# bluescarni/heyoka

Hardware: AMD Instinct MI355X
Metric: ODE systems x steps/sec (fp64) (higher is better)
Workload: dtype f64

## Files before the change

### heyoka_amd/csrc/hip_emit_cluster2.cpp

```cpp
#include <algorithm>
#include <cstdio>
#include <functional>

#include "hip_emit_cluster2_gen.hpp"
#include "logging.hpp"

namespace heyoka_amd::cluster2_detail
{

cluster2_gen::cluster2_gen(const taylor_program &p_, const emit_options &opts_, std::string &why_not_, bool allow_one_lane_,
                           std::uint32_t min_lanes_)
    : c2_emit(p_, opts_.order), p(p_), opts(opts_), why_not(why_not_), allow_one_lane(allow_one_lane_), min_lanes(min_lanes_),
      n_eq(p_.n_eq), order(opts_.order)
{
    std::string s = opts.dev.v5_opts;
    std::replace(s.begin(), s.end(), '+', ',');
    for (std::size_t b = 0, en = 0; b <= s.size(); b = en + 1u) {
        en = std::min(s.find(',', b), s.size());
        v5_flags.insert(s.substr(b, en - b));
    }
}

cluster2_attempt cluster2_gen::run()
{
// ... 93 lines not shown
            for (std::uint32_t i = 0; i < 3u; ++i) {
                pl.slot_of[pl.clusters[c][static_cast<std::uint32_t>(pp.rx[i])]] = static_cast<int>(ns++);
            }
        }
        number_glue_slots(ns);
    }
    L = pl.L, spw = pl.spw;
    bs = pairk ? 512u : 256u;
    wpb = bs / 64u;
    n_ext = static_cast<std::uint32_t>(pl.ext_u[0].size());
    n_out = static_cast<std::uint32_t>(pl.out_pos.size());
    n_cst = static_cast<std::uint32_t>(pl.cst_pos.size());

    variant = one_lane ? cluster2_variant::one_lane : (pair_split ? cluster2_variant::lane_pair : cluster2_variant::pipelined);
    frx = false;
    if (one_lane && !m4 && pp.rx[0] >= 0 && pl.groups.size() == 1u && !v5_flag("nofrx")) {
        auto &nodes = pl.groups[0].nodes;
        std::map<std::uint32_t, bool> is_rx_out;
        for (std::uint32_t c = 0; c < nc; ++c) {
            for (std::uint32_t i = 0; i < 3u; ++i) {
                is_rx_out[pl.clusters[c][pp.pr[i]]] = false;
                is_rx_out[pl.clusters[c][static_cast<std::uint32_t>(pp.rx[i])]] = true;
            }
        }
        const auto &n0 = p.nodes[nodes[0] - n_eq];
        frx = n0.kind == func_kind::sum && n0.args.size() >= 2u;
        std::vector<char> plain(nodes.size(), 1);
        for (std::size_t j = 0; j < nodes.size() && frx; ++j) {
            const auto &nd = p.nodes[nodes[j] - n_eq];
            frx = nd.kind == func_kind::sum && nd.args.size() == n0.args.size();
            for (const auto &o : nd.args) {
                const auto it = is_var(o) ? is_rx_out.find(o.idx) : is_rx_out.end();
                frx = frx && it != is_rx_out.end();
                if (frx && it->second) {
                    plain[j] = 0;
                }
            }
        }
        if (frx) {
            std::vector<std::uint32_t> first, last;
            for (std::size_t j = 0; j < nodes.size(); ++j) {
                (plain[j] != 0 ? last : first).push_back(nodes[j]);
            }
            frx = first.size() <= pl.L && !last.empty();
            if (frx) {
                first.insert(first.end(), last.begin(), last.end());
                nodes = std::move(first);
            }
        }
    }
}

void cluster2_gen::anchors_and_reaction_fusion()
{
    std::vector<int> anchor(n_eq, -1);
    std::vector<std::uint32_t> depth(n_eq, 0);
    for (std::uint32_t i = 0; i < n_eq; ++i) {
        std::uint32_t cur = i, d = 0;
        std::set<std::uint32_t> seen;
        for (;;) {
            if (!seen.insert(cur).second) {
                why_not = "cyclic chain of state-variable definitions";
                return;
            }
// ... 38 lines not shown
    for (std::size_t g = 0; g < pl.groups.size(); ++g) {
        const auto &nodes = pl.groups[g].nodes;
        const auto it0 = att.find(nodes[0]);
        const auto n0 = it0 == att.end() ? 0u : static_cast<std::uint32_t>(it0->second.size());
        for (const auto u : nodes) {
            const auto it = att.find(u);
            const auto n = it == att.end() ? 0u : static_cast<std::uint32_t>(it->second.size());
            if (n != n0) {
                why_not = "glue nodes of one group with different state-variable chains";
                return;
            }
        }
        grp_natt[g] = n0;
    }

    {
        std::uint32_t next = 0;
        for (std::size_t g = 0; g < pl.groups.size(); ++g) {
            const auto &nodes = pl.groups[g].nodes;
            const auto n_nodes = static_cast<std::uint32_t>(nodes.size());
            for (std::uint32_t r = 0; r * L < n_nodes; ++r) {
                for (std::uint32_t a = 0; a < grp_natt[g]; ++a) {
                    for (std::uint32_t l = 0; l < L && r * L + l < n_nodes; ++l) {
                        pl.slot_of[att.at(nodes[r * L + l])[a]] = static_cast<int>(next++);
                    }
                }
            }
        }
        if (next != n_eq) {
            why_not = "internal error: state-variable slots";
            return;
        }
    }

    rx_fused.assign(p.n_u, 0);
    rx_src.assign(p.n_u, 0);
    fuse_rx = false;
    if (pairk && pp.rx[0] >= 0) {
        fuse_rx = !one_lane || frx;
        for (std::size_t c = 0; c < nc; ++c) {
            for (std::uint32_t i = 0; i < 3u; ++i) {
                const auto u = pl.clusters[c][static_cast<std::uint32_t>(pp.rx[i])];
                rx_fused[u] = 1;
                rx_src[u] = pl.clusters[c][pp.pr[i]];
            }
        }
        std::vector<char> in_sum_group(p.n_u, 0);
// ... 11 lines not shown
                if (is_var(o) && rx_fused[o.idx] != 0 && in_sum_group[u] == 0) {
                    fuse_rx = false;
                }
            }
        }
        for (const auto &d : p.sv_defs) {
            if (is_var(d) && rx_fused[d.idx] != 0) {
                fuse_rx = false;
            }
        }
        if (!fuse_rx) {
            std::fill(rx_fused.begin(), rx_fused.end(), 0);
        }
    }
    frx = frx && fuse_rx;
    glue_read.assign(p.n_u, 0);
    for (const auto &n : p.nodes) {
        for (const auto &o : n.args) {
            if (is_var(o)) {
                glue_read[o.idx] = 1;
            }
        }
    }
}

void cluster2_gen::layout_one_lane()
{
    bk_in_slab = one_lane && !v5_flag("nobkslab");
    if (one_lane) {
        for (std::size_t g = 0; g < pl.groups.size(); ++g) {
// ... 106 lines not shown
            }
            if (vexch) {
                vx_col.assign(pl.L, {});
                for (std::uint32_t l = 0; l < pl.L; ++l) {
                    const auto c = l < nc ? l : 0u;
                    for (std::uint32_t sd = 0; sd < 2u; ++sd) {
                        const auto tr = body_vars(c, sd);
                        vx_col[l][sd] = body_col[static_cast<std::size_t>(std::find(bodies.begin(), bodies.end(), tr) - bodies.begin())];
                    }
                }
            }
        }
        const bool wide_an = wide_rd;
        wide_rd = wide_rd && !frx;
        vexch = vexch && wide_an;
        std::vector<int> remap(pl.n_slots, -1);
        std::uint32_t ns = 0;
        const auto keep = [&](std::uint32_t u) {
            if (pl.slot_of[u] < 0) {
                return false;
            }
            if (pl.cluster_of[u] != -1) {
                if (fuse_rx && rx_fused[u] != 0) {
                    return pl.slot_of[rx_src[u]] < 0;
                }
                return true;
            }
            if (vexch && u < n_eq) {
                return false;
            }
// ... 37 lines not shown
                    }
                }
            }
        };
        std::vector<std::vector<std::uint32_t>> rd_pat;
        for (std::uint32_t i = 0; i < 3u; ++i) {
            for (std::uint32_t sd = 0; sd < 2u; ++sd) {
                std::vector<std::uint32_t> v(pl.L);
                for (std::uint32_t l = 0; l < pl.L; ++l) {
                    v[l] = pl.ext_u[l < nc ? l : 0u][pp.de[i][sd]];
                }
                rd_pat.push_back(std::move(v));
            }
        }
        for (const auto &grp : pl.groups) {
            const auto n_nodes = static_cast<std::uint32_t>(grp.nodes.size());
            const auto &n0 = p.nodes[grp.nodes[0] - n_eq];
            for (std::uint32_t r = 0; r * pl.L < n_nodes; ++r) {
                for (std::size_t a = 0; a < n0.args.size(); ++a) {
                    if (!is_var(n0.args[a])) {
                        continue;
                    }
                    std::vector<std::uint32_t> v(pl.L);
                    for (std::uint32_t l = 0; l < pl.L; ++l) {
                        const auto j = r * pl.L + l;
                        v[l] = p.nodes[grp.nodes[j < n_nodes ? j : r * pl.L] - n_eq].args[a].idx;
                        if (fuse_rx && rx_fused[v[l]] != 0) {
                            v[l] = rx_src[v[l]];
                        }
                    }
                    rd_pat.push_back(std::move(v));
                }
            }
        }
        const auto cost = [&](std::uint32_t stride) {
            std::uint64_t tot = 0;
            const auto spw_ = 64u / pl.L;
            for (const auto &v : rd_pat) {
                for (std::uint32_t g = 0; g < 2u; ++g) {
                    std::map<std::uint32_t, std::set<std::uint32_t>> banks;
                    for (std::uint32_t lane = 32u * g; lane < 32u * g + 32u; ++lane) {
// ... 216 lines not shown
    for (std::size_t x = 0; !pairk && x < pl.par_pos.size(); ++x) {
        std::vector<std::uint32_t> v(L);
        for (std::uint32_t l = 0; l < L; ++l) {
            v[l] = pl.par_idx[l < nc ? l : 0u][x];
        }
        const auto [q, a] = pl.par_pos[x];
        e.numpar_override[&p.nodes[t0()[q] - n_eq].args[a]] = lane_par(std::move(v));
    }
}

void cluster2_gen::build_glue_rounds()
{
    rounds.assign(pl.groups.size(), {});
    for (std::size_t g = 0; g < pl.groups.size(); ++g) {
        const auto &grp = pl.groups[g];
        const auto n_nodes = static_cast<std::uint32_t>(grp.nodes.size());
        const auto n_rounds = (n_nodes + L - 1u) / L;
        const auto &n0 = p.nodes[grp.nodes[0] - n_eq];
        for (std::uint32_t r = 0; r < n_rounds; ++r) {
            glue_round gr;
            gr.n_valid = std::min(L, n_nodes - r * L);
            const auto node_of = [&](std::uint32_t l) {
                const auto j = r * L + l;
                return grp.nodes[j < n_nodes ? j : r * L];
            };
            bool round_fused = false;
            for (std::uint32_t l = 0; fuse_rx && l < L; ++l) {
                for (const auto &o : p.nodes[node_of(l) - n_eq].args) {
                    round_fused = round_fused || (is_var(o) && rx_fused[o.idx] != 0);
                }
            }
            for (std::size_t a = 0; a < n0.args.size(); ++a) {
                if (is_var(n0.args[a]) && round_fused) {
                    std::vector<std::uint32_t> v(L);
                    std::vector<double> cf(L, 1.);
                    for (std::uint32_t l = 0; l < L; ++l) {
                        const auto ua = p.nodes[node_of(l) - n_eq].args[a].idx;
                        if (rx_fused[ua] != 0) {
                            v[l] = pr_slot(rx_src[ua], ua, 0);
                            cf[l] = p.nodes[ua - n_eq].args[0].value;
                        } else {
                            v[l] = static_cast<std::uint32_t>(pl.slot_of[ua]);
                        }
                    }
                    gr.arg_tbl.push_back(add_utbl(std::move(v)));
                    gr.coef_tbl.push_back(add_dtbl(std::move(cf)));
                } else if (is_var(n0.args[a])) {
// ... 9 lines not shown
                    }
                    gr.arg_tbl.push_back(add_dtbl(std::move(v)));
                } else {
                    std::vector<std::uint32_t> v(L);
                    for (std::uint32_t l = 0; l < L; ++l) {
                        v[l] = p.nodes[node_of(l) - n_eq].args[a].idx;
                    }
                    gr.par_name.resize(n0.args.size());
                    gr.par_name[a] = lane_par(std::move(v));
                    gr.arg_tbl.push_back(0);
                }
            }
            bool any_read = false;
            std::vector<std::uint32_t> v(L);
            for (std::uint32_t l = 0; l < L; ++l) {
                const auto j = r * L + l;
                v[l] = (j < n_nodes && pl.slot_of[grp.nodes[j]] >= 0) ? static_cast<std::uint32_t>(pl.slot_of[grp.nodes[j]]) : dummy_base;
                any_read = any_read || (j < n_nodes && glue_read[grp.nodes[j]] != 0);
            }
            gr.exported = any_read;
            gr.out_tbl = add_utbl(std::move(v));
            for (std::uint32_t a = 0; a < grp_natt[g]; ++a) {
                owner_slot ow;
                std::vector<std::uint32_t> vs(L), vv(L);
                for (std::uint32_t l = 0; l < L; ++l) {
                    const auto var = att.at(node_of(l))[a];
                    vs[l] = (r * L + l < n_nodes && pl.slot_of[var] >= 0) ? static_cast<std::uint32_t>(pl.slot_of[var]) : dummy_base;
                    vv[l] = var;
                }
                ow.out_tbl = add_utbl(std::move(vs));
                ow.var_tbl = add_utbl(std::move(vv), false);
                ow.col = n_own++;
                ow.n_valid = gr.n_valid;
                if (one_lane && a >= 1u) {
                    ow.derived = true;
                    ow.parent = gr.owners[a - 1u].col;
                    ow.cbase = n_dcol;
                    n_dcol += gr.n_valid;
                } else {
                    ow.cbase = n_col;
                    n_col += gr.n_valid;
                }
                ow.xname.resize(order + 1u);
                ow.slab_needed = false;
                for (std::uint32_t l = 0; l < L && r * L + l < n_nodes; ++l) {
                    ow.slab_needed = ow.slab_needed || glue_read[att.at(grp.nodes[r * L + l])[a]] != 0;
                }
                ow.slab_needed = ow.slab_needed && !vexch;
                gr.owners.push_back(std::move(ow));
            }
            rounds[g].push_back(std::move(gr));
        }
    }
    if (n_own == 0u) {
        why_not = "no state variable could be attached to a glue round";
        return;
    }
}

void cluster2_gen::layout_jets_and_schedule()
{
// ... 146 lines not shown
        if (k >= 1u) {
            for (std::size_t g = 0; g < pl.groups.size(); ++g) {
                for (std::uint32_t r = 0; r < rounds[g].size(); ++r) {
                    pend.emplace_back(g, r, emit_glue_reads(g, r, k - 1u));
                }
            }
        }
        if (one_lane) {
            if (prio_switch) {
                os << "__builtin_amdgcn_s_setprio(3);\n";
            }
            sched_fence();
            if (k < order) {
                sched_fence();
            }
            for (const auto &[g, r, names] : pend) {
                emit_glue_compute(g, r, k - 1u, names);
            }
            if (k < order) {
                emit_single_compute(k, prd);
            }
            if (k < order) {
                emit_single_history(k);
            }
            if (prio_switch && k == order && prio_mode != 2) {
                os << "__builtin_amdgcn_s_setprio(0);\n";
            }
            sync();
            continue;
        }
        if (k < order) {
            emit_pair_compute(k, prd);
// ... 182 lines not shown
    src << "__constant__ unsigned short hy_utbl[" << std::max<std::size_t>(utbl.size(), 1u) * L << "] = {";
    for (const auto &v : utbl) {
        for (const auto x : v) {
            if (x > 65535u) {
                why_not = "slot / variable index overflow in the lane tables";
                return;
            }
            src << x << ",";
        }
    }
    src << "};\n";
    {
        std::vector<std::uint32_t> col_of(n_eq, 0);
        for_each_owner([&](auto &, auto &ow) {
            const auto &vv = utbl[ow.var_tbl];
            for (std::uint32_t l2 = 0; l2 < ow.n_valid; ++l2) {
                col_of[vv[l2]] = ow.cbase + l2;
            }
        });
        if (m4) {
            struct tc_entry {
                std::uint64_t row, off, stride;
            };
            std::vector<tc_entry> tc_src;
            if (one_lane) {
                for_each_owner([&](auto &, auto &ow) {
                    const auto &vv = utbl[ow.var_tbl];
                    for (std::uint32_t l2 = 0; l2 < ow.n_valid; ++l2) {
                        const std::uint64_t var = vv[l2];
                        if (ow.derived) {
                            tc_src.push_back({var * (order + 1u), jet_rows_doubles + jet_off(ow) + l2, jet_sys(ow)});
// ... 99 lines not shown
            src << "const double crs_r = hy_dtbl[" << st1.crs * L << "u + l];\n";
        }
    }
    if (!pk_tbl.empty()) {
        src << "__shared__ double lds_fac[" << 2u * (order + 1u) << "];\n";
        src << "for (unsigned i = threadIdx.x; i < " << 2u * (order + 1u) << "u; i += " << bs << "u) lds_fac[i] = (i <= " << order
            << "u) ? 1.0 : hy_rk[i - " << (order + 1u) << "u];\n__syncthreads();\n";
    }
    for (std::size_t t = 0; !one_lane && t < dtbl.size(); ++t) {
        src << "const double dt" << t << " = hy_dtbl[" << t * L << "u + l];\n";
    }
    for (std::uint32_t x = 0; !pairk && x < n_cst; ++x) {
        src << "const double ccst" << x << " = dt" << cst_tbl[x] << ";\n";
    }
    for_each_owner([&](auto &gr, auto &ow) {
        src << "const bool ovalid" << ow.col << " = l < " << gr.n_valid << "u;\n";
        if (ow.derived) {
            src << "double *const x0c" << ow.col << " = jetw + " << jet_rows_doubles + jet_off(ow) << "u + q * " << jet_sys(ow)
                << "u + (ovalid" << ow.col << " ? l : 0u);\n";
            src << "const double *const x0r" << ow.col << " = x0c" << ow.col << ";\n";
            return;
        }
        if (one_lane) {
            src << "double *const jc" << ow.col << " = jetw + " << jet_off(ow) << "u + q * " << jet_sys(ow) << "u + (ovalid"
                << ow.col << " ? l : 0u);\n";
            src << "const double *const jr" << ow.col << " = jc" << ow.col << ";\n";
            return;
        }
        src << "double *const jc" << ow.col << " = jetw + q * " << n_colp << "u + (ovalid" << ow.col << " ? "
            << ow.cbase << "u + l : " << n_col << "u);\n";
        src << "const double *const jr" << ow.col << " = jetw + q * " << n_colp << "u + " << ow.cbase
            << "u + (ovalid" << ow.col << " ? l : 0u);\n";
    });
    for (std::uint32_t h = 0; !one_lane && h < n_hslots; ++h) {
        src << "double *const hc" << h << " = jetw + q * " << n_colp << "u + ((" << h * L << "u + l < " << n_col << "u) ? "
            << h * L << "u + l : " << n_col << "u);\n";
    }
}

void cluster2_gen::text_event_equations()
{
    ev_inline = false;
    const bool packed_tail_ev = L >= 4u;
    if (m4 && one_lane && jet_lds && packed_tail_ev && opts.ev_prog != nullptr && !opts.exact_division && slab_stride >= n_own * L
        && opts.dev.events_in_stepper) {
        struct sv_loc {
            bool derived = false;
            std::uint64_t off = 0;
// ... 324 lines not shown
        }
        tail_passes.push_back({&ow, dv, dv != nullptr && pk_tbl.count(ow.col) != 0u, {}, {}});
    });
    kstride = static_cast<std::uint64_t>(spw) * n_colp;
    if (one_lane && !m4 && jet_lds && opts.high_accuracy && packed_tail && !v5_flag("notailrd")) {
        src << "// (Jet reads of the final evaluation issued ahead of the selector.)\n";
        const auto hoist = [&](const std::string &ex) {
            auto nm = "trd" + std::to_string(n_trd++);
            src << "const double " << nm << " = " << ex << ";\n";
            return nm;
        };
        for (auto &tp : tail_passes) {
            const auto cs = std::to_string(tp.ow->col);
            if (tp.packed) {
                const auto &tb = pk_tbl.at(tp.ow->col);
                src << "const double *const pk_jh" << cs << " = jetw + q * " << jet_sys(*tp.ow) << "u + hy_utbl[" << tb[1] * L << "u + l];\n";
                src << "const double *const pk_fh" << cs << " = lds_fac + hy_utbl[" << tb[2] * L << "u + l];\n";
                tp.rows.resize(order + 1u);
                tp.facs.resize(order + 1u);
                for (std::uint32_t k = 1; k <= order; ++k) {
                    tp.rows[k] = hoist("pk_jh" + cs + "[" + std::to_string((k - 1u) * kstride) + "]");
                    tp.facs[k] = hoist("pk_fh" + cs + "[" + std::to_string(k) + "]");
                }
            } else {
                for (std::uint32_t k = 0; k <= order; ++k) {
                    tp.rows.push_back(hoist("jr" + cs + "[" + std::to_string(k * kstride) + "]"));
                }
            }
        }
        src << "__builtin_amdgcn_sched_barrier(0);\n";
    }
    if (packed_tail) {
// ... 105 lines not shown
void cluster2_gen::text_final_evaluation_and_update()
{
    src << "asm volatile(\"\" ::: \"memory\");\n";
    const char *jet_fence = jet_lds ? "" : "__builtin_amdgcn_fence(__ATOMIC_SEQ_CST, \"wavefront\");\n";
    src << jet_fence;
    std::vector<std::tuple<std::string, std::string, std::string>> upd;
    for (const auto &tp : tail_passes) {
        const auto &ow = *tp.ow;
        const auto *const dv = tp.dv;
        const auto xn = "xn" + std::to_string(ow.col);
        const auto xd = dv != nullptr ? "xn" + std::to_string(dv->col) : std::string{};
        const auto colp = "jr" + std::to_string(ow.col);
        if (tp.packed) {
            const auto cs = std::to_string(ow.col);
            const auto &tb = pk_tbl.at(ow.col);
            src << "double *const pk_v" << cs << " = jetw + q * " << jet_sys(ow) << "u + hy_utbl[" << tb[0] * L << "u + l];\n";
            src << "double " << xn << ";\n{\n";
            if (tp.rows.empty()) {
                src << "const double *const pk_j = jetw + q * " << jet_sys(ow) << "u + hy_utbl[" << tb[1] * L << "u + l];\n";
                src << "const double *const pk_f = lds_fac + hy_utbl[" << tb[2] * L << "u + l];\n";
            }
            src << "double res = pk_v" << cs << "[0], comp = 0.0, cur_h = h;\n";
            for (std::uint32_t k = 1; k <= order; ++k) {
                src << "{\nconst double ck = " << tail_val(tp.rows, k, "pk_j[" + std::to_string((k - 1u) * kstride) + "]") << " * "
                    << tail_val(tp.facs, k, "pk_f[" + std::to_string(k) + "]") << ";\n"
                    << "const double tmp = ck * cur_h;\nconst double y = tmp - comp;\nconst double t = res + y;\n"
                    << "comp = (t - res) - y;\nres = t;\n";
                if (k < order) {
                    src << "cur_h = cur_h * h;\n";
                }
                src << "}\n";
// ... 314 lines not shown
    res.mod.cluster_mode4 = m4;
    res.mod.events_in_stepper = ev_inline;
    res.mod.compact_tc = compact_tc;
    res.mod.tc_by_threshold = one_lane && jet_lds && !m4;
    res.mod.grid_multi_step = res.mod.tc_by_threshold;
    res.jets_in_lds = one_lane && jet_lds;
    res.variant = variant;
    res.mod.cluster_generation = one_lane ? 5 : (pair_split ? 3 : 2);
    res.mod.notes = std::string(one_lane ? "cluster mode v5 (one lane per pair, 2 wavefronts per SIMD): "
                                     : (pair_split ? "cluster mode v3 (lane pairs, 2 wavefronts per SIMD): " : "cluster mode v2 (pipelined): "))
                + std::to_string(nc) + " clusters of " + std::to_string(t0().size())
                + " nodes, L=" + std::to_string(L) + ", " + std::to_string(pl.n_slots) + " LDS slots x2, "
                + std::to_string(n_own) + " state-variable owner slots, " + std::to_string(utbl.size())
                + " slot tables, jets in " + (jet_lds ? "LDS" : "global scratch")
                + (one_lane ? ", slab layout: " + std::to_string(bank_cost) + " conflict cycles per step in the model" : std::string{})
                + (ev_inline ? "; event equations, final step size and state update inside the stepper" : "");
}

}
namespace heyoka_amd
{

emitted_module emit_cluster_v2(const taylor_program &p, const emit_options &opts, std::string &why_not)
{
    std::string why1;
    const bool try_one_lane = opts.cluster_kernel == 0 || opts.cluster_kernel == 5;
    for (const std::uint32_t min_lanes : {4u, 8u, 16u}) {
        why1.clear();
        auto at = cluster2_detail::cluster2_gen(p, opts, why1, try_one_lane, min_lanes).run();
        const bool is_v5 = why1.empty() && at.variant == cluster2_detail::cluster2_variant::one_lane, in_lds = at.jets_in_lds;
// ... 17 lines not shown
```

### heyoka_amd/csrc/hip_emit_cluster2_gen.hpp

```cpp
#pragma once

#include <array>
#include <map>
#include <set>
#include <tuple>

#include "hip_emit_cluster_plan.hpp"
#include "hip_emit_detail.hpp"

namespace heyoka_amd::cluster2_detail
{

using cluster_detail::cluster_plan;
using cluster_detail::is_var;
using emit_detail::prelude;
using emit_detail::rhofac;
using emit_detail::ssa_emitter;
using psel = ssa_emitter::part_sel;

enum class cluster2_variant { pipelined, lane_pair, one_lane };

struct cluster2_attempt {
    emitted_module mod;
    cluster2_variant variant = cluster2_variant::pipelined;
    bool jets_in_lds = false;
    bool more_lanes_cure = false;
};

struct c2_variant {
    cluster2_variant variant = cluster2_variant::pipelined;
    bool one_lane = false, pair_split = false;
    bool pairk = false;
    bool m4 = false;
    bool frx = false;
    bool fuse_rx = false;
    bool frx_regs = false, merged = false;
    std::set<std::string> v5_flags;
    bool v5_flag(const char *name) const { return v5_flags.count(name) != 0u; }
};

struct c2_geometry {
    cluster_plan pl;
    cluster_detail::pair_pattern pp;
    std::vector<char> cu;
    std::uint32_t nc = 0, L = 0, spw = 0, bs = 0, wpb = 0, n_ext = 0, n_out = 0, n_cst = 0;
    const std::vector<std::uint32_t> &t0() const { return pl.clusters[0]; }
    std::array<std::uint32_t, 3> body_vars(std::uint32_t c, std::uint32_t sd) const
    {
        return {pl.ext_u[c][pp.de[0][sd]], pl.ext_u[c][pp.de[1][sd]], pl.ext_u[c][pp.de[2][sd]]};
    }
};

struct owner_slot {
    std::size_t out_tbl = 0;
    std::size_t var_tbl = 0;
    std::uint32_t col = 0;
    std::uint32_t cbase = 0;
    std::uint32_t n_valid = 0;
    std::vector<std::string> xname;
    bool slab_needed = true;
    bool derived = false;
    std::uint32_t parent = 0;
};
struct glue_round {
    std::vector<std::size_t> arg_tbl;
    std::size_t out_tbl = 0;
    std::uint32_t n_valid = 0;
    bool exported = true;
    std::vector<owner_slot> owners;
    std::vector<std::string> par_name;
    std::vector<std::string> c0name;
    std::vector<std::size_t> coef_tbl;
};

struct c2_layout {
    std::map<std::uint32_t, std::vector<std::uint32_t>> att;
    std::vector<std::uint32_t> grp_natt;
    std::vector<char> rx_fused;
    std::vector<std::uint32_t> rx_src;
    std::vector<char> glue_read;
    std::vector<std::uint32_t> lane_pr, lane_rx;
    bool wide_rd = false;
    bool vexch = false;
    std::vector<std::array<std::uint32_t, 2>> vx_col;
    std::vector<std::array<std::uint32_t, 3>> wide_pr, wide_rx;
    std::uint32_t slab_stride_opt = 0;
    std::uint64_t bank_cost = 0;
    bool bk_in_slab = false;
    std::vector<std::array<std::uint32_t, 3>> bodies;
    std::vector<std::uint32_t> node_coord, node_rank;
    std::uint32_t n_rank = 0, n_args = 0;
    std::uint32_t dummy_base = 0, n_slots_tot = 0, buf_stride = 0, slab_stride = 0;
    std::vector<std::vector<glue_round>> rounds;
    std::uint32_t n_own = 0;
    std::uint32_t n_col = 0;
    std::uint32_t n_colp = 0;
    std::uint32_t n_dcol = 0, n_dcolp = 0;
    std::uint32_t n_hslots = 0;
    std::uint64_t jet_rows_doubles = 0, jet_doubles_per_wave = 0;
    bool jet_lds = false, compact_tc = false;
    std::size_t n_tc_rows = 0;
};

struct c2_tables {
    std::vector<std::vector<std::uint32_t>> utbl;
    std::vector<std::vector<double>> dtbl;
// ... 52 lines not shown
struct cluster2_gen : c2_variant, c2_geometry, c2_layout, c2_tables, c2_emit {
    const taylor_program &p;
    const emit_options &opts;
    std::string &why_not;
    const bool allow_one_lane;
    const std::uint32_t min_lanes, n_eq, order;
    cluster2_attempt res;

    cluster2_gen(const taylor_program &p, const emit_options &opts, std::string &why_not, bool allow_one_lane, std::uint32_t min_lanes);
    cluster2_attempt run();

    void plan_and_select_variant(), anchors_and_reaction_fusion(), layout_one_lane(), lds_layout_and_lane_tables(),
        build_glue_rounds(), layout_jets_and_schedule(), init_order_programs(), emit_step_body(),
        text_helpers_and_constant_tables(), text_kernel_prologue(), text_event_equations(), text_pickup(), text_selector(),
        text_event_exclusion(), text_final_evaluation_and_update(), text_refill_and_tail(), finish();
    void number_glue_slots(std::uint32_t ns), place_wide_read_slots();
    template <typename F>
    void for_each_owner(F &&f)
    {
        for (auto &rg : rounds) {
            for (auto &gr : rg) {
                for (auto &ow : gr.owners) {
                    f(gr, ow);
                }
            }
        }
    }

    std::size_t add_utbl(std::vector<std::uint32_t> v, bool is_slot = true);
    std::size_t add_dtbl(std::vector<double> v);
    std::string utname(std::size_t t) const { return utexpr[t]; }
// ... 32 lines not shown
```

### heyoka_amd/csrc/hip_emit_cluster2_layout.cpp

```cpp
#include <algorithm>
#include <cstdio>
#include <functional>

#include "hip_emit_cluster2_gen.hpp"

namespace heyoka_amd::cluster2_detail
{

void cluster2_gen::place_wide_read_slots()
{
    const auto W = (n_args + 2u) & ~1u;
    const auto nb = static_cast<std::uint32_t>(bodies.size());
    const auto &grp = pl.groups[0];
    struct lds_op {
        int width;
        std::vector<std::uint32_t> addr;
    };
    const auto pos_sz = vexch ? 0u : 4u * nb;
    std::uint32_t Dd = W * n_rank, pos_base = 0, op_base = pos_sz;
    std::vector<std::vector<std::uint32_t>> arr_pos(n_rank, std::vector<std::uint32_t>(n_args));
    for (std::uint32_t r = 0; r < n_rank; ++r) {
        for (std::uint32_t a = 0; a < n_args; ++a) {
            arr_pos[r][a] = W * r + a;
        }
// ... 297 lines not shown
                const auto rp = l < nc ? pr_ref[l][i] : ~0u, rr = l < nc ? rx_ref[l][i] : ~0u;
                wide_pr[l][i] = rp != ~0u ? ref_slot(rp) : dummy_pr(i);
                wide_rx[l][i] = rr != ~0u ? ref_slot(rr) : dummy_rx(i);
                if (l < nc && rp != ~0u) {
                    pl.slot_of[pl.clusters[l][pp.pr[i]]] = static_cast<int>(wide_pr[l][i]);
                }
                if (l < nc && rr != ~0u) {
                    pl.slot_of[pl.clusters[l][static_cast<std::uint32_t>(pp.rx[i])]] = static_cast<int>(wide_rx[l][i]);
                }
            }
        }
        pl.n_slots = total_for(Dd) - 2u - (bk_in_slab ? 16u : 0u);
    }
}

std::size_t cluster2_gen::add_utbl(std::vector<std::uint32_t> v, bool is_slot)
{
    for (std::size_t t = 0; t < utbl.size(); ++t) {
        if (utbl[t] == v && (utbl_is_slot[t] != 0) == is_slot) {
            return t;
        }
    }
    std::string ex = "ut" + std::to_string(utbl.size());
    for (std::size_t t = 0; one_lane && is_slot && t < utbl.size(); ++t) {
        if (utbl_is_slot[t] == 0 || utexpr[t] != "ut" + std::to_string(t)) {
            continue;
        }
        const auto d = static_cast<std::int64_t>(v[0]) - static_cast<std::int64_t>(utbl[t][0]);
        bool affine = true;
        for (std::size_t l2 = 0; l2 < v.size(); ++l2) {
// ... 44 lines not shown
```

### heyoka_amd/csrc/hip_emit_cluster2_orders.cpp

```cpp
#include <cstdio>

#include "hip_emit_cluster2_gen.hpp"

namespace heyoka_amd::cluster2_detail
{

std::string cluster2_gen::slabk(std::uint32_t k, const std::string &tbl) const
{
    return (k % 2u == 0u || buf_stride == 0u) ? ("slab[" + tbl + "]")
                                              : ("slab[" + tbl + " + " + std::to_string(buf_stride) + "u]");
}

void cluster2_gen::publish_sv(owner_slot &ow, std::uint32_t k, const std::string &name)
{
    ow.xname[k] = name;
    if (ow.slab_needed) {
        os << slabk(k, utname(ow.out_tbl)) << " = " << name << ";\n";
    }
    if (k != 0u && !ow.derived) {
        os << jet_at(k, ow.col) << " = " << name << ";\n";
    }
    const char *acc = (k == 0u) ? "m0" : (k == order ? "mo" : (k == order - 1u ? "mom1" : nullptr));
    if (acc != nullptr) {
        os << acc << " = hy_nmax(" << acc << ", fabs(" << name << "));\n";
    }
}

std::string cluster2_gen::wide_read(const std::string &tbl)
{
    const auto nm = "w" + std::to_string(n_wide++);
    os << "const hy_d2 " << nm << " = *reinterpret_cast<const hy_d2 *>(slab + " << tbl << ");\n";
    ++e.n_stmt;
    return nm;
}

std::vector<std::string> cluster2_gen::emit_glue_reads(std::size_t g, std::uint32_t r, std::uint32_t k)
{
    const auto &grp = pl.groups[g];
    auto &gr = rounds[g][r];
    const auto &n0 = p.nodes[grp.nodes[0] - n_eq];
    std::vector<std::string> names(n0.args.size());
    for (std::size_t a = 0; a < n0.args.size(); ++a) {
        if (wide_rd && a + 1u < n0.args.size() && a % 2u == 0u) {
            const auto w = wide_read(utname(gr.arg_tbl[a]));
            names[a] = w + ".x";
            names[a + 1u] = w + ".y";
            ++a;
            continue;
        }
        if (is_var(n0.args[a])) {
            names[a] = e.def(slabk(k, utname(gr.arg_tbl[a])));
        }
    }
    return names;
}

void cluster2_gen::emit_glue_compute(std::size_t g, std::uint32_t r, std::uint32_t k, const std::vector<std::string> &names)
{
    const auto &grp = pl.groups[g];
    auto &gr = rounds[g][r];
    const auto rep = grp.nodes[0];
    const auto &n0 = p.nodes[rep - n_eq];
    const auto saved = e.numpar_override;
    std::vector<std::pair<std::uint32_t, std::string>> saved_vals, saved_vals0;
    std::string fused_val;
    if (!gr.coef_tbl.empty()) {
        std::vector<std::string> terms;
        for (std::size_t a = 0; a + 1u < names.size(); a += 2u) {
            const auto m = e.def(ssa_emitter::mul(coefname(gr.coef_tbl[a + 1u]), names[a + 1u]));
            terms.push_back(e.def("__builtin_fma(" + coefname(gr.coef_tbl[a]) + ", " + names[a] + ", " + m + ")"));
        }
        const bool odd = names.size() % 2u == 1u;
        while (terms.size() > 1u) {
            std::vector<std::string> nt;
            for (std::size_t i = 0; i + 1u < terms.size(); i += 2u) {
                nt.push_back(e.def(terms[i] + " + " + terms[i + 1u]));
            }
            if (terms.size() % 2u == 1u) {
                nt.push_back(terms.back());
            }
            terms = std::move(nt);
// ... 396 lines not shown
```

Measured before the change: 812.3 million.

## Reduce later five-term sums across first-round lanes with DPP instead of extra round

In the one-lane pair kernel with fused reactions, the glue nodes of the second round (five-term sums of first-round outputs) are computed by a cross-lane DPP reduction over the lanes that produce their terms. The lanes are reordered so each sum's terms sit in adjacent lanes, and unused second-round stores are parked on columns the first round overwrites. This removes a full glue round of slab reads per Taylor order and replaces it with a few DPP shuffle-adds. In exchange it adds lane-mapping tables, per-lane jet pointers computed through table lookups, and a more complex slot numbering.

```diff
diff --git a/heyoka_amd/csrc/hip_emit_cluster2.cpp b/heyoka_amd/csrc/hip_emit_cluster2.cpp
--- a/heyoka_amd/csrc/hip_emit_cluster2.cpp
+++ b/heyoka_amd/csrc/hip_emit_cluster2.cpp
@@ -131,6 +131,7 @@
 
     variant = one_lane ? cluster2_variant::one_lane : (pair_split ? cluster2_variant::lane_pair : cluster2_variant::pipelined);
     frx = false;
+    lane_sum = false;
     if (one_lane && !m4 && pp.rx[0] >= 0 && pl.groups.size() == 1u && !v5_flag("nofrx")) {
         auto &nodes = pl.groups[0].nodes;
         std::map<std::uint32_t, bool> is_rx_out;
@@ -161,10 +162,34 @@
             }
             frx = first.size() <= pl.L && !last.empty();
             if (frx) {
+                const auto n_first = static_cast<std::uint32_t>(first.size());
                 first.insert(first.end(), last.begin(), last.end());
                 nodes = std::move(first);
-            }
-        }
+                if (!v5_flag("nolanesum")) {
+                    plan_lane_sums(n_first);
+                }
+            }
+        }
+    }
+}
+
+void cluster2_gen::renumber_sv_slots()
+{
+    std::uint32_t next = 0;
+    for (std::size_t g = 0; g < pl.groups.size(); ++g) {
+        const auto &nodes = pl.groups[g].nodes;
+        for (std::uint32_t r = 0; r < n_rounds_of(g); ++r) {
+            for (std::uint32_t a = 0; a < grp_natt[g]; ++a) {
+                for (std::uint32_t l = 0; l < L; ++l) {
+                    if (const auto [j, valid] = round_node(g, r, l); valid) {
+                        pl.slot_of[att.at(nodes[j])[a]] = static_cast<int>(next++);
+                    }
+                }
+            }
+        }
+    }
+    if (next != n_eq) {
+        why_not = "internal error: state-variable slots";
     }
 }
 
@@ -233,23 +258,9 @@
         grp_natt[g] = n0;
     }
 
-    {
-        std::uint32_t next = 0;
-        for (std::size_t g = 0; g < pl.groups.size(); ++g) {
-            const auto &nodes = pl.groups[g].nodes;
-            const auto n_nodes = static_cast<std::uint32_t>(nodes.size());
-            for (std::uint32_t r = 0; r * L < n_nodes; ++r) {
-                for (std::uint32_t a = 0; a < grp_natt[g]; ++a) {
-                    for (std::uint32_t l = 0; l < L && r * L + l < n_nodes; ++l) {
-                        pl.slot_of[att.at(nodes[r * L + l])[a]] = static_cast<int>(next++);
-                    }
-                }
-            }
-        }
-        if (next != n_eq) {
-            why_not = "internal error: state-variable slots";
-            return;
-        }
+    renumber_sv_slots();
+    if (!why_not.empty()) {
+        return;
     }
 
     rx_fused.assign(p.n_u, 0);
@@ -291,6 +302,13 @@
         }
     }
     frx = frx && fuse_rx;
+    if (lane_sum && !frx) {
+        lane_sum = false;
+        renumber_sv_slots();
+        if (!why_not.empty()) {
+            return;
+        }
+    }
     glue_read.assign(p.n_u, 0);
     for (const auto &n : p.nodes) {
         for (const auto &o : n.args) {
@@ -427,6 +445,10 @@
         const bool wide_an = wide_rd;
         wide_rd = wide_rd && !frx;
         vexch = vexch && wide_an;
+        if (lane_sum && !vexch) {
+            lane_sum = false;
+            renumber_sv_slots();
+        }
         std::vector<int> remap(pl.n_slots, -1);
         std::uint32_t ns = 0;
         const auto keep = [&](std::uint32_t u) {
@@ -494,17 +516,16 @@
             }
         }
         for (const auto &grp : pl.groups) {
-            const auto n_nodes = static_cast<std::uint32_t>(grp.nodes.size());
+            const auto g = static_cast<std::size_t>(&grp - pl.groups.data());
             const auto &n0 = p.nodes[grp.nodes[0] - n_eq];
-            for (std::uint32_t r = 0; r * pl.L < n_nodes; ++r) {
+            for (std::uint32_t r = 0; r < (lane_sum && g == 0u ? 1u : n_rounds_of(g)); ++r) {
                 for (std::size_t a = 0; a < n0.args.size(); ++a) {
                     if (!is_var(n0.args[a])) {
                         continue;
                     }
                     std::vector<std::uint32_t> v(pl.L);
                     for (std::uint32_t l = 0; l < pl.L; ++l) {
-                        const auto j = r * pl.L + l;
-                        v[l] = p.nodes[grp.nodes[j < n_nodes ? j : r * pl.L] - n_eq].args[a].idx;
+                        v[l] = p.nodes[grp.nodes[round_node(g, r, l).first] - n_eq].args[a].idx;
                         if (fuse_rx && rx_fused[v[l]] != 0) {
                             v[l] = rx_src[v[l]];
                         }
@@ -751,23 +772,26 @@
     rounds.assign(pl.groups.size(), {});
     for (std::size_t g = 0; g < pl.groups.size(); ++g) {
         const auto &grp = pl.groups[g];
-        const auto n_nodes = static_cast<std::uint32_t>(grp.nodes.size());
-        const auto n_rounds = (n_nodes + L - 1u) / L;
+        const auto n_rounds = n_rounds_of(g);
         const auto &n0 = p.nodes[grp.nodes[0] - n_eq];
         for (std::uint32_t r = 0; r < n_rounds; ++r) {
             glue_round gr;
-            gr.n_valid = std::min(L, n_nodes - r * L);
-            const auto node_of = [&](std::uint32_t l) {
-                const auto j = r * L + l;
-                return grp.nodes[j < n_nodes ? j : r * L];
-            };
+            const bool mapped = lane_sum && g == 0u;
+            std::uint32_t valid_mask = 0;
+            for (std::uint32_t l = 0; l < L; ++l) {
+                valid_mask |= round_node(g, r, l).second ? (1u << l) : 0u;
+            }
+            const auto is_valid = [&](std::uint32_t l) { return (valid_mask >> l & 1u) != 0u; };
+            gr.n_valid = static_cast<std::uint32_t>(__builtin_popcount(valid_mask));
+            gr.reduced = mapped && r == 1u;
+            const auto node_of = [&](std::uint32_t l) { return grp.nodes[round_node(g, r, l).first]; };
             bool round_fused = false;
             for (std::uint32_t l = 0; fuse_rx && l < L; ++l) {
                 for (const auto &o : p.nodes[node_of(l) - n_eq].args) {
                     round_fused = round_fused || (is_var(o) && rx_fused[o.idx] != 0);
                 }
             }
-            for (std::size_t a = 0; a < n0.args.size(); ++a) {
+            for (std::size_t a = 0; a < n0.args.size() && !gr.reduced; ++a) {
                 if (is_var(n0.args[a]) && round_fused) {
                     std::vector<std::uint32_t> v(L);
                     std::vector<double> cf(L, 1.);
@@ -807,9 +831,9 @@
             bool any_read = false;
             std::vector<std::uint32_t> v(L);
             for (std::uint32_t l = 0; l < L; ++l) {
-                const auto j = r * L + l;
-                v[l] = (j < n_nodes && pl.slot_of[grp.nodes[j]] >= 0) ? static_cast<std::uint32_t>(pl.slot_of[grp.nodes[j]]) : dummy_base;
-                any_read = any_read || (j < n_nodes && glue_read[grp.nodes[j]] != 0);
+                const auto u = node_of(l);
+                v[l] = (is_valid(l) && pl.slot_of[u] >= 0) ? static_cast<std::uint32_t>(pl.slot_of[u]) : dummy_base;
+                any_read = any_read || (is_valid(l) && glue_read[u] != 0);
             }
             gr.exported = any_read;
             gr.out_tbl = add_utbl(std::move(v));
@@ -818,8 +842,18 @@
                 std::vector<std::uint32_t> vs(L), vv(L);
                 for (std::uint32_t l = 0; l < L; ++l) {
                     const auto var = att.at(node_of(l))[a];
-                    vs[l] = (r * L + l < n_nodes && pl.slot_of[var] >= 0) ? static_cast<std::uint32_t>(pl.slot_of[var]) : dummy_base;
+                    vs[l] = (is_valid(l) && pl.slot_of[var] >= 0) ? static_cast<std::uint32_t>(pl.slot_of[var]) : dummy_base;
                     vv[l] = var;
+                }
+                if (mapped) {
+                    std::vector<std::uint32_t> vc(L);
+                    for (std::uint32_t l = 0; l < L; ++l) {
+                        vc[l] = round_node(g, r, l).first;
+                    }
+                    ow.mapped = true;
+                    ow.reduced = gr.reduced;
+                    ow.col_tbl = add_utbl(std::move(vc), false);
+                    ow.valid_mask = valid_mask;
                 }
                 ow.out_tbl = add_utbl(std::move(vs));
                 ow.var_tbl = add_utbl(std::move(vv), false);
@@ -836,8 +870,8 @@
                 }
                 ow.xname.resize(order + 1u);
                 ow.slab_needed = false;
-                for (std::uint32_t l = 0; l < L && r * L + l < n_nodes; ++l) {
-                    ow.slab_needed = ow.slab_needed || glue_read[att.at(grp.nodes[r * L + l])[a]] != 0;
+                for (std::uint32_t l = 0; l < L; ++l) {
+                    ow.slab_needed = ow.slab_needed || (is_valid(l) && glue_read[att.at(node_of(l))[a]] != 0);
                 }
                 ow.slab_needed = ow.slab_needed && !vexch;
                 gr.owners.push_back(std::move(ow));
@@ -1014,8 +1048,13 @@
             if (k < order) {
                 sched_fence();
             }
-            for (const auto &[g, r, names] : pend) {
-                emit_glue_compute(g, r, k - 1u, names);
+            if (lane_sum && k >= 1u) {
+                emit_glue_compute(0, 1, k - 1u, {std::get<2>(pend[0]).at(ls_pos)});
+                emit_glue_compute(0, 0, k - 1u, std::get<2>(pend[0]));
+            } else {
+                for (const auto &[g, r, names] : pend) {
+                    emit_glue_compute(g, r, k - 1u, names);
+                }
             }
             if (k < order) {
                 emit_single_compute(k, prd);
@@ -1228,7 +1267,12 @@
         std::vector<std::uint32_t> col_of(n_eq, 0);
         for_each_owner([&](auto &, auto &ow) {
             const auto &vv = utbl[ow.var_tbl];
-            for (std::uint32_t l2 = 0; l2 < ow.n_valid; ++l2) {
+            for (std::uint32_t l2 = 0; l2 < L && ow.mapped; ++l2) {
+                if ((ow.valid_mask >> l2 & 1u) != 0u) {
+                    col_of[vv[l2]] = utbl[ow.col_tbl][l2];
+                }
+            }
+            for (std::uint32_t l2 = 0; l2 < ow.n_valid && !ow.mapped; ++l2) {
                 col_of[vv[l2]] = ow.cbase + l2;
             }
         });
@@ -1358,6 +1402,14 @@
         src << "const double ccst" << x << " = dt" << cst_tbl[x] << ";\n";
     }
     for_each_owner([&](auto &gr, auto &ow) {
+        if (ow.mapped) {
+            src << "const bool ovalid" << ow.col << " = ((" << ow.valid_mask << "u >> l) & 1u) != 0u;\n";
+            const auto nm = (ow.derived ? "x0c" : "jc") + std::to_string(ow.col);
+            src << "double *const " << nm << " = jetw + " << (ow.derived ? jet_rows_doubles : 0u) << "u + q * " << jet_sys(ow)
+                << "u + hy_utbl[" << ow.col_tbl * L << "u + l];\n";
+            src << "const double *const " << (ow.derived ? "x0r" : "jr") << ow.col << " = " << nm << ";\n";
+            return;
+        }
         src << "const bool ovalid" << ow.col << " = l < " << gr.n_valid << "u;\n";
         if (ow.derived) {
             src << "double *const x0c" << ow.col << " = jetw + " << jet_rows_doubles + jet_off(ow) << "u + q * " << jet_sys(ow)
@@ -1376,6 +1428,18 @@
         src << "const double *const jr" << ow.col << " = jetw + q * " << n_colp << "u + " << ow.cbase
             << "u + (ovalid" << ow.col << " ? l : 0u);\n";
     });
+    for (const auto &[col, tb] : pk_tbl) {
+        if (!lane_sum) {
+            break;
+        }
+        for_each_owner([&, col = col, tb = tb](auto &, auto &ow) {
+            if (ow.col == col) {
+                src << "const double *const pk_jh" << col << " = jetw + q * " << jet_sys(ow) << "u + hy_utbl[" << tb[1] * L << "u + l];\n";
+                src << "const double *const pk_fh" << col << " = lds_fac + hy_utbl[" << tb[2] * L << "u + l];\n";
+                src << "double *const pk_v" << col << " = jetw + q * " << jet_sys(ow) << "u + hy_utbl[" << tb[0] * L << "u + l];\n";
+            }
+        });
+    }
     for (std::uint32_t h = 0; !one_lane && h < n_hslots; ++h) {
         src << "double *const hc" << h << " = jetw + q * " << n_colp << "u + ((" << h * L << "u + l < " << n_col << "u) ? "
             << h * L << "u + l : " << n_col << "u);\n";
@@ -1730,8 +1794,10 @@
             const auto cs = std::to_string(tp.ow->col);
             if (tp.packed) {
                 const auto &tb = pk_tbl.at(tp.ow->col);
-                src << "const double *const pk_jh" << cs << " = jetw + q * " << jet_sys(*tp.ow) << "u + hy_utbl[" << tb[1] * L << "u + l];\n";
-                src << "const double *const pk_fh" << cs << " = lds_fac + hy_utbl[" << tb[2] * L << "u + l];\n";
+                if (!lane_sum) {
+                    src << "const double *const pk_jh" << cs << " = jetw + q * " << jet_sys(*tp.ow) << "u + hy_utbl[" << tb[1] * L << "u + l];\n";
+                    src << "const double *const pk_fh" << cs << " = lds_fac + hy_utbl[" << tb[2] * L << "u + l];\n";
+                }
                 tp.rows.resize(order + 1u);
                 tp.facs.resize(order + 1u);
                 for (std::uint32_t k = 1; k <= order; ++k) {
@@ -1867,7 +1933,9 @@
         if (tp.packed) {
             const auto cs = std::to_string(ow.col);
             const auto &tb = pk_tbl.at(ow.col);
-            src << "double *const pk_v" << cs << " = jetw + q * " << jet_sys(ow) << "u + hy_utbl[" << tb[0] * L << "u + l];\n";
+            if (!lane_sum) {
+                src << "double *const pk_v" << cs << " = jetw + q * " << jet_sys(ow) << "u + hy_utbl[" << tb[0] * L << "u + l];\n";
+            }
             src << "double " << xn << ";\n{\n";
             if (tp.rows.empty()) {
                 src << "const double *const pk_j = jetw + q * " << jet_sys(ow) << "u + hy_utbl[" << tb[1] * L << "u + l];\n";
@@ -2212,6 +2280,7 @@
                 + std::to_string(n_own) + " state-variable owner slots, " + std::to_string(utbl.size())
                 + " slot tables, jets in " + (jet_lds ? "LDS" : "global scratch")
                 + (one_lane ? ", slab layout: " + std::to_string(bank_cost) + " conflict cycles per step in the model" : std::string{})
+                + (lane_sum ? ", later sums reduced across the lanes of the first round" : "")
                 + (ev_inline ? "; event equations, final step size and state update inside the stepper" : "");
 }
 
diff --git a/heyoka_amd/csrc/hip_emit_cluster2_gen.hpp b/heyoka_amd/csrc/hip_emit_cluster2_gen.hpp
--- a/heyoka_amd/csrc/hip_emit_cluster2_gen.hpp
+++ b/heyoka_amd/csrc/hip_emit_cluster2_gen.hpp
@@ -35,6 +35,7 @@
     bool frx = false;
     bool fuse_rx = false;
     bool frx_regs = false, merged = false;
+    bool lane_sum = false;
     std::set<std::string> v5_flags;
     bool v5_flag(const char *name) const { return v5_flags.count(name) != 0u; }
 };
@@ -61,6 +62,9 @@
     bool slab_needed = true;
     bool derived = false;
     std::uint32_t parent = 0;
+    bool mapped = false, reduced = false;
+    std::size_t col_tbl = 0;
+    std::uint32_t valid_mask = 0;
 };
 struct glue_round {
     std::vector<std::size_t> arg_tbl;
@@ -71,6 +75,7 @@
     std::vector<std::string> par_name;
     std::vector<std::string> c0name;
     std::vector<std::size_t> coef_tbl;
+    bool reduced = false;
 };
 
 struct c2_layout {
@@ -90,6 +95,8 @@
     std::vector<std::array<std::uint32_t, 3>> bodies;
     std::vector<std::uint32_t> node_coord, node_rank;
     std::uint32_t n_rank = 0, n_args = 0;
+    std::vector<std::uint32_t> ls_first, ls_last, ls_park;
+    std::uint32_t ls_pos = 0;
     std::uint32_t dummy_base = 0, n_slots_tot = 0, buf_stride = 0, slab_stride = 0;
     std::vector<std::vector<glue_round>> rounds;
     std::uint32_t n_own = 0;
@@ -172,7 +179,9 @@
         build_glue_rounds(), layout_jets_and_schedule(), init_order_programs(), emit_step_body(),
         text_helpers_and_constant_tables(), text_kernel_prologue(), text_event_equations(), text_pickup(), text_selector(),
         text_event_exclusion(), text_final_evaluation_and_update(), text_refill_and_tail(), finish();
-    void number_glue_slots(std::uint32_t ns), place_wide_read_slots();
+    void number_glue_slots(std::uint32_t ns), place_wide_read_slots(), plan_lane_sums(std::uint32_t n_first), renumber_sv_slots();
+    std::uint32_t n_rounds_of(std::size_t g) const;
+    std::pair<std::uint32_t, bool> round_node(std::size_t g, std::uint32_t r, std::uint32_t l) const;
     template <typename F>
     void for_each_owner(F &&f)
     {
diff --git a/heyoka_amd/csrc/hip_emit_cluster2_layout.cpp b/heyoka_amd/csrc/hip_emit_cluster2_layout.cpp
--- a/heyoka_amd/csrc/hip_emit_cluster2_layout.cpp
+++ b/heyoka_amd/csrc/hip_emit_cluster2_layout.cpp
@@ -335,6 +335,114 @@
     }
 }
 
+void cluster2_gen::plan_lane_sums(std::uint32_t n_first)
+{
+    constexpr std::uint32_t n_terms = 5;
+    const auto &nodes = pl.groups[0].nodes;
+    const auto n_nodes = static_cast<std::uint32_t>(nodes.size());
+    if (n_nodes <= L || n_first >= n_nodes || n_first > L) {
+        return;
+    }
+    std::map<std::uint32_t, std::uint32_t> raw_of;
+    for (std::uint32_t c = 0; c < nc; ++c) {
+        for (std::uint32_t i = 0; i < 3u; ++i) {
+            raw_of[pl.clusters[c][pp.pr[i]]] = pl.clusters[c][pp.pr[i]];
+            raw_of[pl.clusters[c][static_cast<std::uint32_t>(pp.rx[i])]] = pl.clusters[c][pp.pr[i]];
+        }
+    }
+    std::map<std::uint32_t, std::pair<std::uint32_t, std::uint32_t>> holder;
+    std::set<std::uint32_t> shared;
+    for (std::uint32_t j = 0; j < n_first; ++j) {
+        const auto &args = p.nodes[nodes[j] - n_eq].args;
+        for (std::uint32_t a = 0; a < args.size(); ++a) {
+            const auto u = raw_of.at(args[a].idx);
+            if (!holder.emplace(u, std::make_pair(j, a)).second) {
+                shared.insert(u);
+            }
+        }
+    }
+    std::vector<std::uint32_t> first_lanes, last_lanes;
+    std::vector<char> taken(n_first, 0);
+    std::uint32_t pos = ~0u;
+    for (std::uint32_t j = n_first; j < n_nodes; ++j) {
+        const auto &args = p.nodes[nodes[j] - n_eq].args;
+        const auto l0 = static_cast<std::uint32_t>(first_lanes.size());
+        if (args.size() != n_terms || l0 % 16u + n_terms > std::min(L, 16u)) {
+            return;
+        }
+        for (const auto &o : args) {
+            const auto it = holder.find(o.idx);
+            if (it == holder.end() || shared.count(o.idx) != 0u || taken[it->second.first] != 0
+                || (pos != ~0u && it->second.second != pos)) {
+                return;
+            }
+            pos = it->second.second;
+            taken[it->second.first] = 1;
+            first_lanes.push_back(it->second.first);
+        }
+        last_lanes.push_back(l0 + n_terms - 1u);
+    }
+    for (std::uint32_t j = 0; j < n_first; ++j) {
+        if (taken[j] == 0) {
+            first_lanes.push_back(j);
+        }
+    }
+    ls_first.assign(L, ~0u);
+    ls_last.assign(L, ~0u);
+    std::copy(first_lanes.begin(), first_lanes.end(), ls_first.begin());
+    for (std::size_t s = 0; s < last_lanes.size(); ++s) {
+        ls_last[last_lanes[s]] = n_first + static_cast<std::uint32_t>(s);
+    }
+    ls_pos = pos;
+    ls_park.assign(L, ~0u);
+    std::set<std::uint32_t> banks;
+    for (const auto j : ls_last) {
+        if (j != ~0u) {
+            banks.insert(j % 16u);
+        }
+    }
+    for (std::uint32_t l = 0; l < L; ++l) {
+        if (ls_last[l] == ~0u && ls_first[l] != ~0u && banks.insert(ls_first[l] % 16u).second) {
+            ls_park[l] = ls_first[l];
+        }
+    }
+    for (std::uint32_t l = 0; l < L; ++l) {
+        for (std::uint32_t j = 0; ls_last[l] == ~0u && ls_park[l] == ~0u && j < n_first; ++j) {
+            if (banks.insert(j % 16u).second) {
+                ls_park[l] = j;
+            }
+        }
+        if (ls_last[l] == ~0u && ls_park[l] == ~0u) {
+            ls_park[l] = ls_first[l] != ~0u ? ls_first[l] : ls_first[0];
+        }
+    }
+    for (std::uint32_t l = 0; l < L; ++l) {
+        if (ls_last[l] == ~0u && std::find(first_lanes.begin(), first_lanes.end(), ls_park[l]) == first_lanes.end()) {
+            throw std::logic_error("hy_taylor (one lane per pair): a store of the lane-reduced round is parked on a column which "
+                                   "the first round does not overwrite");
+        }
+    }
+    lane_sum = true;
+}
+
+std::uint32_t cluster2_gen::n_rounds_of(std::size_t g) const
+{
+    return (lane_sum && g == 0u) ? 2u : (static_cast<std::uint32_t>(pl.groups[g].nodes.size()) + L - 1u) / L;
+}
+
+std::pair<std::uint32_t, bool> cluster2_gen::round_node(std::size_t g, std::uint32_t r, std::uint32_t l) const
+{
+    if (lane_sum && g == 0u) {
+        if (r == 1u) {
+            return ls_last[l] != ~0u ? std::make_pair(ls_last[l], true) : std::make_pair(ls_park[l], false);
+        }
+        return ls_first[l] != ~0u ? std::make_pair(ls_first[l], true) : std::make_pair(ls_first[0], false);
+    }
+    const auto n_nodes = static_cast<std::uint32_t>(pl.groups[g].nodes.size());
+    const auto j = r * L + l;
+    return j < n_nodes ? std::make_pair(j, true) : std::make_pair(r * L, false);
+}
+
 std::size_t cluster2_gen::add_utbl(std::vector<std::uint32_t> v, bool is_slot)
 {
     for (std::size_t t = 0; t < utbl.size(); ++t) {
diff --git a/heyoka_amd/csrc/hip_emit_cluster2_orders.cpp b/heyoka_amd/csrc/hip_emit_cluster2_orders.cpp
--- a/heyoka_amd/csrc/hip_emit_cluster2_orders.cpp
+++ b/heyoka_amd/csrc/hip_emit_cluster2_orders.cpp
@@ -21,7 +21,9 @@
         os << jet_at(k, ow.col) << " = " << name << ";\n";
     }
     const char *acc = (k == 0u) ? "m0" : (k == order ? "mo" : (k == order - 1u ? "mom1" : nullptr));
-    if (acc != nullptr) {
+    if (acc != nullptr && ow.reduced && k != 0u) {
+        os << acc << " = hy_nmax(" << acc << ", fabs(ovalid" << ow.col << " ? " << name << " : 0.0));\n";
+    } else if (acc != nullptr) {
         os << acc << " = hy_nmax(" << acc << ", fabs(" << name << "));\n";
     }
 }
@@ -40,7 +42,7 @@
     auto &gr = rounds[g][r];
     const auto &n0 = p.nodes[grp.nodes[0] - n_eq];
     std::vector<std::string> names(n0.args.size());
-    for (std::size_t a = 0; a < n0.args.size(); ++a) {
+    for (std::size_t a = 0; a < n0.args.size() && !gr.reduced; ++a) {
         if (wide_rd && a + 1u < n0.args.size() && a % 2u == 0u) {
             const auto w = wide_read(utname(gr.arg_tbl[a]));
             names[a] = w + ".x";
@@ -64,7 +66,12 @@
     const auto saved = e.numpar_override;
     std::vector<std::pair<std::uint32_t, std::string>> saved_vals, saved_vals0;
     std::string fused_val;
-    if (!gr.coef_tbl.empty()) {
+    if (gr.reduced) {
+        const auto &t = names.at(0);
+        const auto sa = e.def(t + " + hy_dpp<0x111>(" + t + ")");
+        const auto sb = e.def(sa + " + hy_dpp<0x112>(" + sa + ")");
+        fused_val = e.def(t + " + hy_dpp<0x111>(" + sb + ")");
+    } else if (!gr.coef_tbl.empty()) {
         std::vector<std::string> terms;
         for (std::size_t a = 0; a + 1u < names.size(); a += 2u) {
             const auto m = e.def(ssa_emitter::mul(coefname(gr.coef_tbl[a + 1u]), names[a + 1u]));
```

After: 834.6 million, median of 6. +2.7%, better.
